# iliasam/STM32F4_SDR_GPS

Hardware: AMD Instinct MI355X
Metric: acquisition hypotheses/sec (PRN x Doppler x phase) (higher is better)
Workload: dtype u1 (MX-FP4 operands, exact f32 accumulation)

## Files before the change

stm32f4_sdr_gps_amd/csrc/k_acq_mx.hip:

```cpp
#if !defined(GPSX_LAB) && defined(MX_VARIANT_B)
#error "variants of k_acq_mx for same-box A/B timing build with -DGPSX_LAB only: tools/build_variant.sh"
#endif
#include <cstdlib>

#include "gpsx_device.hpp"
#include "gpsx_kernels.hpp"

namespace gpsx {

namespace {

typedef int v8i __attribute__((ext_vector_type(8)));
typedef int v4i __attribute__((ext_vector_type(4)));
typedef float v16f __attribute__((ext_vector_type(16)));

constexpr int kMxThreads = 512;
constexpr int kMxTiles = 4;
constexpr int kCopyDwords = 260;
constexpr int kVecDwords = 258;
constexpr int kPlaneWordsMx = 66;
constexpr u32 kScaleOne = 0x7F7F7F7Fu;
constexpr u32 kScaleA = 0x72727272u;
constexpr float kAccScale = 1.0f / 8192.0f;
constexpr float kUnscaleSq = 67108864.0f;
constexpr u32 kScaleEight = 0x82828282u;
constexpr int kPasses = 17;

struct MxShared {
  uint16_t x[1024];
  u32 d[2][514];
  u32 plane[2][16][kPlaneWordsMx];
  u32 base[2][kCopyDwords];
  u32 e8[2][2][8][kCopyDwords];
  u32 corr[2][2][2][128];
  v4i chips_a[16][2][32];
  u32 chip_t[1032];
  u32 ones[2];
  u32 t_lut[768];
  alignas(16) u32 part[8][32][2][32];
};

__device__ __forceinline__ v8i widen(v4i x) { return v8i{x.x, x.y, x.z, x.w, 0, 0, 0, 0}; }

__device__ __forceinline__ u32 lds_byte(const u32 *words, int byte_index)
{
  return (words[byte_index >> 2] >> ((byte_index & 3) * 8)) & 0xFFu;
}

__device__ __forceinline__ u32 spread8(u32 x)
{
  u32 t = (x | (x << 12)) & 0x000F000Fu;
  t = (t | (t << 6)) & 0x03030303u;
  t = (t | (t << 3)) & 0x11111111u;
  return t;
}

__device__ __forceinline__ int wrap1023(int i)
{
  i = i >= 2 * kChips ? i - 2 * kChips : i;
  return i >= kChips ? i - kChips : i;
}

__device__ __forceinline__ u32 plane_bits9(const u32 *pl, int pos)
{
  return __builtin_amdgcn_alignbit(pl[(pos >> 5) + 1], pl[pos >> 5], (u32)(pos & 31)) & 0x1FFu;
}

__device__ __forceinline__ void mx_load_block(MxShared &sh, const uint8_t *blk, int if_format, int tid)
{
  for (int i = tid; i < 1024; i += kMxThreads)
    sh.x[i] = i < kWords16 ? load_sign16(blk, i, if_format) : (uint16_t)0;
  if (tid < 2)
    sh.ones[tid] = 0;
}
__device__ void mx_wipe_block(MxShared &sh, u32 step_word, int tid, int lane)
{
  {
    const u32 *x32 = reinterpret_cast<const u32 *>(sh.x);
    u32 ones_i = 0, ones_q = 0;
    for (int w = tid; w < 514; w += kMxThreads) {
      u32 vi = 0, vq = 0;
      if (w < kWords32) {
        const u32 quad = (step_word * (u32)w) >> 30;
        vi = carrier_i(quad) ^ x32[w];
        vq = carrier_q(quad) ^ x32[w];
      }
      sh.d[0][w] = vi;
      sh.d[1][w] = vq;
      ones_i += __popc(vi);
      ones_q += __popc(vq);
    }
    ones_i = wave_sum_to_lane63(ones_i);
    ones_q = wave_sum_to_lane63(ones_q);
    if (lane == 63) {
      atomicAdd(&sh.ones[0], ones_i);
      atomicAdd(&sh.ones[1], ones_q);
    }
  }
  __syncthreads();
  if (tid < 2)
    sh.d[tid][511] = sh.d[tid][0] << 16;
  __syncthreads();
  for (int m = tid; m < 2 * 32 * 16; m += kMxThreads) {
    const int t0 = m & 15, w = (m >> 4) & 31, iq = m >> 9;
    const u32 *src = &sh.d[iq][16 * w];
    u32 bits = 0;
#pragma unroll
    for (int k = 0; k < 16; k++) {
      const u32 sk = src[k];
      bits |= ((sk >> t0) & 1u) << (2 * k);
      bits |= ((sk >> (16 + t0)) & 1u) << (2 * k + 1);
    }
    sh.plane[iq][t0][w] = bits;
  }
  __syncthreads();
  for (int m = tid; m < 2 * 16 * (kPlaneWordsMx - 32); m += kMxThreads) {
    const int w = 32 + m % (kPlaneWordsMx - 32);
    const int r = m / (kPlaneWordsMx - 32);
    const u32 *pl = sh.plane[r >> 4][r & 15];
    const int pos = 32 * w - (w >= 64 ? 2 * kChips : kChips);
    const int lo = pos >> 5;
    u32 v = __builtin_amdgcn_alignbit(lo < 31 ? pl[lo + 1] : 0u, pl[lo], (u32)(pos & 31));
    if (pos + 32 > kChips) {
      const int k = kChips - pos;
      v = (v & ((1u << k) - 1u)) | (pl[0] << k);
    }
    sh.plane[r >> 4][r & 15][w] = v;
  }
}

__device__ __forceinline__ u32 fp4_code(int v)
{
  const u32 m = (u32)(v < 0 ? -v : v);
  return ((0x0765420u >> (4u * (m > 5u ? 5u : m))) & 0xFu) | (v < 0 ? 8u : 0u);
}

__device__ void mx_fill_tables(MxShared &sh, int tid)
{
  for (int w = tid; w < 512; w += kMxThreads) {
    const u32 cur = (u32)w & 0xFFu, nxt = ((u32)w >> 1) & 0xFFu;
    const u32 plus = spread8(nxt & ~cur), minus = spread8(cur & ~nxt);
    sh.t_lut[w] = (plus << 2) | (plus << 3) | (minus << 2);
  }
  for (int x = tid; x < 256; x += kMxThreads)
    sh.t_lut[512 + x] = (spread8((u32)x) << 1) | (spread8(~(u32)x & 0xFFu) * 0xAu);
}

__device__ void mx_vector_phase1(MxShared &sh, int pass, int buf, int tid, int nthreads)
{
  const int t0 = pass - 1;
  for (int m = tid; m < 2 * kVecDwords + 2 * 128; m += nthreads) {
    if (m < 2 * kVecDwords) {
      const int iq = m >= kVecDwords, dw = m - iq * kVecDwords;
      u32 packed = 0;
      if (pass < 2) {
        const u32 *dd = sh.d[iq];
#pragma unroll
        for (int e = 0; e < 8; e++) {
          const int k = wrap1023(8 * dw + e);
          const int pos = 16 * k;
          const u32 sum = pop16(__builtin_amdgcn_alignbit(dd[(pos >> 5) + 1], dd[pos >> 5], (u32)(pos & 31)));
          const u32 code = pass == 0 ? (0xFEC0u >> (4u * (sum & 3u))) & 0xFu : (0xEDCA0u >> (4u * (sum >> 2))) & 0xFu;
          packed |= code << (4 * e);
        }
      } else {
        const u32 w = plane_bits9(sh.plane[iq][pass - 2], 8 * dw);
        packed = sh.t_lut[w];
        if (dw == 127 && t0 >= 9) {
          const u32 cur = w & 0xFFu, nxt = (w >> 1) & 0xFFu;
          const int e5 = (int)((nxt >> 5) & 1u) - (int)((cur >> 5) & 1u), e6 = (int)((nxt >> 6) & 1u) - (int)((cur >> 6) & 1u);
          packed = (packed & ~0x0FF00000u) | (fp4_code(-2 * e5 - 1) << 20) | (fp4_code(-2 * e6 + 1) << 24);
        }
      }
      sh.base[iq][dw] = packed;
    } else {
      const int mm = m - 2 * kVecDwords;
      const int iq = mm >> 7, dw = mm & 127;
      u32 ca = 0, cb = 0;
      if (pass >= 2 && t0 != 8) {
        const u32 *pl = sh.plane[iq][pass - 2];
        const u32 w = dw ? plane_bits9(pl, 8 * dw - 1) : (pl[0] << 1) & 0x1FFu;
        const u32 exist = dw == 127 ? 0x0FFFFFFFu : 0xFFFFFFFFu;
        if (t0 < 8) {
          ca = sh.t_lut[512 + (w >> 1)] & exist;
        } else {
          const u32 diff = sh.t_lut[w];
          ca = (diff ^ ((diff & 0x44444444u) << 1)) & exist;
          cb = sh.t_lut[512 + (w & 0xFFu)] & exist;
          if (dw == 0) {
            ca = (ca & ~0xFu) | ((w & 2u) ? 0x2u : 0xAu);
            cb &= ~0xFu;
          }
        }
      }
      sh.corr[buf][iq][0][dw] = ca;
      sh.corr[buf][iq][1][dw] = cb;
    }
  }
}

__device__ void mx_vector_phase2(MxShared &sh, int buf, int tid, int nthreads)
{
  for (int m = tid; m < 2 * 256; m += nthreads) {
    const int iq = m >> 8, j = m & 255;
    const u32 lo = sh.base[iq][j], hi = sh.base[iq][j + 1];
#pragma unroll
    for (int c = 0; c < 8; c++)
      sh.e8[buf][iq][c][j] = c ? __builtin_amdgcn_alignbit(hi, lo, 4u * (u32)c) : lo;
  }
}

typedef __attribute__((address_space(3))) const u32 lds_cu32;

__device__ __forceinline__ lds_cu32 *lds_opaque(const u32 *p)
{
  u32 a = (u32)(size_t)(lds_cu32 *)p;
  asm volatile("" : "+v"(a));
  return (lds_cu32 *)(size_t)a;
}
__device__ __forceinline__ v4i lds_frag(lds_cu32 *w, int dw)
{
  return v4i{(int)w[dw], (int)w[dw + 1], (int)w[dw + 2], (int)w[dw + 3]};
}

__device__ __forceinline__ u32 mx_patch_wrap(u32 packed, u32 w9, bool patch)
{
  const u32 i5 = 1u + ((w9 >> 6) & 1u) - ((w9 >> 5) & 1u), i6 = 1u + ((w9 >> 7) & 1u) - ((w9 >> 6) & 1u);
  const u32 c5 = (0xDA2u >> (4u * i5)) & 0xFu;
  const u32 c6 = (0xA25u >> (4u * i6)) & 0xFu;
  const u32 patched = (packed & ~0x0FF00000u) | (c5 << 20) | (c6 << 24);
  return patch ? patched : packed;
}

__device__ __forceinline__ void mx_vector_build(MxShared &sh, int p_vec, int tid)
{
  const int t0 = p_vec - 1, buf = p_vec & 1;
  const bool late = t0 >= 9;
  const int iq = tid >> 8, j = tid & 255, which = (tid >> 7) & 1, dwc = tid & 127;
  const u32 *pl = sh.plane[iq][p_vec - 2];
  const u32 x = __builtin_amdgcn_alignbit(pl[(j >> 2) + 1], pl[j >> 2], 8u * (u32)(j & 3));
  const int pos = dwc ? 8 * dwc - 1 : 0;
  const u32 y = __builtin_amdgcn_alignbit(pl[(pos >> 5) + 1], pl[pos >> 5], (u32)(pos & 31));
  const u32 cw = (dwc ? y : y << 1) & 0x1FFu;
  u32 lo = sh.t_lut[x & 0x1FFu], hi = sh.t_lut[(x >> 8) & 0x1FFu];
  u32 v = sh.t_lut[which ? 512u + (cw & 0xFFu) : (late ? cw : 512u + (cw >> 1))];
  if (late) {
    lo = mx_patch_wrap(lo, x & 0x1FFu, j == 127);
    hi = mx_patch_wrap(hi, (x >> 8) & 0x1FFu, j == 126);
    if (which == 0)
      v ^= (v & 0x44444444u) << 1;
    if (dwc == 0)
      v = (v & ~0xFu) | (which ? 0u : ((cw & 2u) ? 0x2u : 0xAu));
  }
  v &= dwc == 127 ? 0x0FFFFFFFu : 0xFFFFFFFFu;
  if ((which && !late) || t0 == 8)
    v = 0;
  sh.corr[buf][iq][which][dwc] = v;
  u32 *dst = &sh.e8[buf][iq][0][j];
#pragma unroll
  for (int c = 0; c < 8; c++)
    dst[c * kCopyDwords] = c ? __builtin_amdgcn_alignbit(hi, lo, 4u * (u32)c) : lo;
}

__device__ __forceinline__ void mx_vector_build_direct(MxShared &sh, int which, int t0s, u32 *e8_dst, int tid)
{
  const int iq = tid >> 8, j = tid & 255;
  const u32 *dd = sh.d[iq];
  u32 w2[2] = {0, 0};
#pragma unroll
  for (int e = 0; e < 16; e++) {
    const int k = wrap1023(8 * j + e);
    const int pos = 16 * k + t0s;
    const u32 sum = pop16(__builtin_amdgcn_alignbit(dd[(pos >> 5) + 1], dd[pos >> 5], (u32)(pos & 31)));
    const u32 code = which == 0 ? (0xFEC0u >> (4u * (sum & 3u))) & 0xFu : (0xEDCA0u >> (4u * (sum >> 2))) & 0xFu;
    w2[e >> 3] |= code << (4 * (e & 7));
  }
  u32 *dst = e8_dst + (iq * 8) * kCopyDwords + j;
#pragma unroll
  for (int c = 0; c < 8; c++)
    dst[c * kCopyDwords] = c ? __builtin_amdgcn_alignbit(w2[1], w2[0], 4u * (u32)c) : w2[0];
}

template <int S, int NT, u32 SCALE_A = kScaleA>
__device__ __forceinline__ void mx_pass_step(lds_cu32 *wi, lds_cu32 *wq, const v4i *ca, v4i (&a)[16], v4i &fi, v4i &fq,
                                             v16f (&acc)[2][NT], u32 scale_b)
{
  constexpr int kSteps = 16 + NT - 1;
  constexpr bool more = S + 1 < kSteps;
  v4i fi_next = fi, fq_next = fq;
  if constexpr (more) {
    fi_next = lds_frag(wi, 8 * (S + 1));
    fq_next = lds_frag(wq, 8 * (S + 1));
    if constexpr (S + 1 < 16)
      a[S + 1] = ca[(S + 1) * 64];
  }
  constexpr int j_lo = S - 15 > 0 ? S - 15 : 0, j_hi = S < NT - 1 ? S : NT - 1;
#pragma unroll
  for (int j = j_lo; j <= j_hi; j++) {
    acc[0][j] = __builtin_amdgcn_mfma_scale_f32_32x32x64_f8f6f4(widen(a[S - j]), widen(fi), acc[0][j], 4, 4, 0, SCALE_A, 0, scale_b);
    acc[1][j] = __builtin_amdgcn_mfma_scale_f32_32x32x64_f8f6f4(widen(a[S - j]), widen(fq), acc[1][j], 4, 4, 0, SCALE_A, 0, scale_b);
  }
  if constexpr (more) {
    __builtin_amdgcn_sched_group_barrier(0x100, S + 1 < 16 ? 5 : 4, 0);
    __builtin_amdgcn_sched_group_barrier(0x008, 2 * (j_hi - j_lo + 1), 0);
  }
  __builtin_amdgcn_sched_barrier(0);
  fi = fi_next;
  fq = fq_next;
  if constexpr (more)
    mx_pass_step<S + 1, NT, SCALE_A>(wi, wq, ca, a, fi, fq, acc, scale_b);
}

template <int S, int NT>
__device__ __forceinline__ void mx_pass_step_inplace(lds_cu32 *wi, lds_cu32 *wq, const v4i *ca, v4i (&a)[16], v4i &fi, v4i &fq,
                                                     v16f (&acc)[2][NT], u32 scale_b)
{
  constexpr int kSteps = 16 + NT - 1;
  constexpr bool more = S + 1 < kSteps;
  if constexpr (more && S + 1 < 16)
    a[S + 1] = ca[(S + 1) * 64];
  constexpr int j_lo = S - 15 > 0 ? S - 15 : 0, j_hi = S < NT - 1 ? S : NT - 1;
#pragma unroll
  for (int j = j_lo; j <= j_hi; j++)
    acc[0][j] = __builtin_amdgcn_mfma_scale_f32_32x32x64_f8f6f4(widen(a[S - j]), widen(fi), acc[0][j], 4, 4, 0, kScaleA, 0, scale_b);
  if constexpr (more)
    fi = lds_frag(wi, 8 * (S + 1));
#pragma unroll
  for (int j = j_lo; j <= j_hi; j++)
    acc[1][j] = __builtin_amdgcn_mfma_scale_f32_32x32x64_f8f6f4(widen(a[S - j]), widen(fq), acc[1][j], 4, 4, 0, kScaleA, 0, scale_b);
  if constexpr (more)
    fq = lds_frag(wq, 8 * (S + 1));
  if constexpr (more) {
    if constexpr (S + 1 < 16)
      __builtin_amdgcn_sched_group_barrier(0x100, 1, 0);
    __builtin_amdgcn_sched_group_barrier(0x008, j_hi - j_lo + 1, 0);
    __builtin_amdgcn_sched_group_barrier(0x100, 2, 0);
    __builtin_amdgcn_sched_group_barrier(0x008, j_hi - j_lo + 1, 0);
    __builtin_amdgcn_sched_group_barrier(0x100, 2, 0);
  }
  __builtin_amdgcn_sched_barrier(0);
  if constexpr (more)
    mx_pass_step_inplace<S + 1, NT>(wi, wq, ca, a, fi, fq, acc, scale_b);
}

template <int S, int NT>
__device__ __forceinline__ void mx_pass2_step(lds_cu32 *const (&w)[4], const v4i *ca, v4i (&a)[16], v4i (&f)[4], v16f (&acc)[2][NT])
{
  constexpr int kSteps = 16 + NT - 1;
  constexpr bool more = S + 1 < kSteps;
  if constexpr (more && S + 1 < 16)
    a[S + 1] = ca[(S + 1) * 64];
  constexpr int j_lo = S - 15 > 0 ? S - 15 : 0, j_hi = S < NT - 1 ? S : NT - 1;
#pragma unroll
  for (int v = 0; v < 4; v++) {
#pragma unroll
    for (int j = j_lo; j <= j_hi; j++)
      acc[v & 1][j] = __builtin_amdgcn_mfma_scale_f32_32x32x64_f8f6f4(widen(a[S - j]), widen(f[v]), acc[v & 1][j], 4, 4, 0, kScaleA, 0,
                                                                      v < 2 ? kScaleOne : kScaleEight);
    if constexpr (more)
      f[v] = lds_frag(w[v], 8 * (S + 1));
  }
  if constexpr (more) {
    if constexpr (S + 1 < 16)
      __builtin_amdgcn_sched_group_barrier(0x100, 1, 0);
#pragma unroll
    for (int v = 0; v < 4; v++) {
      __builtin_amdgcn_sched_group_barrier(0x008, j_hi - j_lo + 1, 0);
      __builtin_amdgcn_sched_group_barrier(0x100, 2, 0);
    }
  }
  __builtin_amdgcn_sched_barrier(0);
  if constexpr (more)
    mx_pass2_step<S + 1, NT>(w, ca, a, f, acc);
}
template <int NT>
__device__ __forceinline__ void mx_pass2(const MxShared &sh, int lane, int q0_tile, v16f (&acc)[2][NT], const u32 *e8_low,
                                         const u32 *e8_high)
{
  const int n = lane & 31, h = lane >> 5;
  const int off = (n & 7) * kCopyDwords + 4 * (q0_tile + h) + (n >> 3);
  lds_cu32 *const w[4] = {lds_opaque(e8_low + off), lds_opaque(e8_low + 8 * kCopyDwords + off), lds_opaque(e8_high + off),
                          lds_opaque(e8_high + 8 * kCopyDwords + off)};
  const v4i *ca = &sh.chips_a[0][h][n];
  v4i a[16];
  v4i f[4] = {lds_frag(w[0], 0), lds_frag(w[1], 0), lds_frag(w[2], 0), lds_frag(w[3], 0)};
  a[0] = ca[0];
  mx_pass2_step<0, NT>(w, ca, a, f, acc);
}

template <bool AHEAD, int NT, u32 SCALE_A = kScaleA>
__device__ __forceinline__ void mx_pass(const MxShared &sh, int buf, int lane, int q0_tile, v16f (&acc)[2][NT],
                                        u32 scale_b, v4i a_corr, bool with_corr, const u32 *e8_buf = nullptr)
{
  const int n = lane & 31, h = lane >> 5;
  const u32 *e8 = e8_buf ? e8_buf : &sh.e8[buf][0][0][0];
  lds_cu32 *wi = lds_opaque(e8 + (n & 7) * kCopyDwords + 4 * (q0_tile + h) + (n >> 3));
  lds_cu32 *wq = lds_opaque(e8 + (8 + (n & 7)) * kCopyDwords + 4 * (q0_tile + h) + (n >> 3));
  const v4i *ca = &sh.chips_a[0][h][n];
  v4i a[16];
  if constexpr (AHEAD) {
    v4i fi = lds_frag(wi, 0), fq = lds_frag(wq, 0);
    a[0] = ca[0];
    mx_pass_step<0, NT, SCALE_A>(wi, wq, ca, a, fi, fq, acc, scale_b);
  } else {
    static_assert(SCALE_A == kScaleA, "the in-place walk is the sign-only grid's");
    v4i fi = lds_frag(wi, 0), fq = lds_frag(wq, 0);
    a[0] = ca[0];
    mx_pass_step_inplace<0, NT>(wi, wq, ca, a, fi, fq, acc, scale_b);
  }
  if (with_corr) {
    lds_cu32 *cw = lds_opaque(&sh.corr[buf][0][h][4 * q0_tile + (n >> 3)]);
#pragma unroll
    for (int j = 0; j < NT; j++) {
      const v4i gi = v4i{(int)(cw[8 * j] >> (4 * (n & 7))), 0, 0, 0};
      const v4i gq = v4i{(int)(cw[8 * j + 2 * 128] >> (4 * (n & 7))), 0, 0, 0};
      acc[0][j] = __builtin_amdgcn_mfma_scale_f32_32x32x64_f8f6f4(widen(a_corr), widen(gi), acc[0][j], 4, 4, 0, kScaleA, 0,
                                                                   kScaleOne);
      acc[1][j] = __builtin_amdgcn_mfma_scale_f32_32x32x64_f8f6f4(widen(a_corr), widen(gq), acc[1][j], 4, 4, 0, kScaleA, 0,
                                                                   kScaleOne);
    }
  }
}

__device__ __forceinline__ u32 root_trunc(float e);
__device__ __forceinline__ float mx_clip_square(float c)
{
  return __builtin_amdgcn_fmed3f(c * __builtin_fabsf(c), 0.0f, 1.0f);
}
__device__ __forceinline__ float clip_square_sum(float ci, float cq)
{
  return mx_clip_square(ci) + mx_clip_square(cq);
}
__device__ __forceinline__ u32 mag8_f32(float ci, float cq)
{
  return root_trunc(clip_square_sum(ci, cq) * kUnscaleSq);
// ... 440 lines not shown
  const int n = lane & 31, h = lane >> 5;
  const int b = t0 & 7, half = t0 >> 3;
  u32 *slot = &sh.part[slots < 0 ? b : slots][4 * h][0][n];
  u32 best[16], total[16];
  u32 kqh[NT];
#pragma unroll
  for (int j = 0; j < NT; j++)
    kqh[j] = kq[j] - (u32)half;
#pragma unroll
  for (int r = 0; r < 16; r++) {
    best[r] = 0;
    total[r] = 0u - (u32)NT * kRootBias;
  }
  mx_round_toward_zero();
#pragma unroll
  for (int jp = 0; jp < NT; jp += 2) {
#pragma unroll
    for (int r0 = 0; r0 < 16; r0 += 4) {
      float ev[8];
      u32 e_max = 0;
#pragma unroll
      for (int i = 0; i < 8; i++) {
        ev[i] = clip_square_sum(acc[0][jp + (i >> 2)][r0 + (i & 3)], acc[1][jp + (i >> 2)][r0 + (i & 3)]);
        e_max = max(e_max, __float_as_uint(ev[i]));
      }
      const bool small = __builtin_amdgcn_ballot_w64(e_max >= 0x3C800000u ) == 0;
      u32 bits[8];
      if (__builtin_expect(small, 1)) {
#pragma unroll
        for (int i = 0; i < 8; i++)
          bits[i] = root_bits_small(ev[i]);
      } else {
        float ci[8], cq[8];
#pragma unroll
        for (int i = 0; i < 8; i++) {
          ci[i] = acc[0][jp + (i >> 2)][r0 + (i & 3)];
          cq[i] = acc[1][jp + (i >> 2)][r0 + (i & 3)];
        }
        mx_roots_exact<8>(ci, cq, bits);
#pragma unroll
        for (int i = 0; i < 8; i++)
          bits[i] += kRootBias;
      }
#pragma unroll
      for (int rr = 0; rr < 4; rr++) {
        const int r = r0 + rr;
        const u32 k0 = (bits[rr] << 11) | kqh[jp], k1 = (bits[4 + rr] << 11) | kqh[jp + 1];
        best[r] = max(max(best[r], k0), k1);
        total[r] = total[r] + bits[rr] + bits[4 + rr];
      }
#pragma unroll
      for (int rr = 0; rr < 4; rr++)
        asm volatile("" : "+v"(best[r0 + rr]), "+v"(total[r0 + rr]));
      __builtin_amdgcn_sched_barrier(0);
    }
  }
  mx_round_to_nearest();
#pragma unroll
  for (int r = 0; r < 16; r++) {
    const int p_off = ((r & 3) + 8 * (r >> 2)) * 64;
    atomicMax(slot + p_off, best[r]);
    atomicAdd(slot + p_off + 32, total[r]);
  }
}

__device__ __forceinline__ void mx_epilogue_store(int lane, int q0_tile, int t0, const v16f (&acc)[2][kMxTiles], u32 group_mask,
                                                  uint16_t *__restrict__ plane0, size_t prn_stride, int slot0, int n_prn)
{
  const int n = lane & 31, h = lane >> 5;
#pragma unroll
  for (int j = 0; j < kMxTiles; j++) {
    const int q = 32 * (q0_tile + 2 * j) + n;
    uint16_t *v = plane0 + (size_t)t0 * 1024 + (size_t)(q & 3) * 256 + (size_t)(q >> 2);
#pragma unroll
    for (int g = 0; g < 4; g++) {
#pragma unroll
      for (int rr = 0; rr < 4; rr++) {
        const int r = 4 * g + rr;
        const int p = (r & 3) + 8 * (r >> 2) + 4 * h;
        const u32 val = mag8_f32(acc[0][j][r], acc[1][j][r]);
        if (((group_mask >> g) & 1u) && slot0 + p < n_prn)
          v[(size_t)p * prn_stride] = (uint16_t)val;
      }
      __builtin_amdgcn_sched_barrier(0);
    }
  }
}



__device__ __forceinline__ unsigned long long mx_max8_u64(unsigned long long v)
{
  u32 lo = (u32)v, hi = (u32)(v >> 32);
#define MX_MAX8(ctrl)                                                                           \
  {                                                                                             \
    const u32 lo2 = (u32)__builtin_amdgcn_mov_dpp((int)lo, ctrl, 0xF, 0xF, true);               \
    const u32 hi2 = (u32)__builtin_amdgcn_mov_dpp((int)hi, ctrl, 0xF, 0xF, true);               \
    const bool g = hi2 > hi || (hi2 == hi && lo2 > lo);                                         \
    lo = g ? lo2 : lo;                                                                          \
    hi = g ? hi2 : hi;                                                                          \
  }
  MX_MAX8(0xB1)
  MX_MAX8(0x4E)
  MX_MAX8(0x141)
#undef MX_MAX8
  return ((unsigned long long)hi << 32) | lo;
}

constexpr int kMxSingle = 0, kMxWalk = 1, kMxStore = 2, kMxWalk16 = 3, kMxByte = 4, kMxSplit = 5;

}

__global__ void k_build_mx_tables(const u32 *__restrict__ chipbits, int n_slots, u32 *__restrict__ mx_a, u32 *__restrict__ mx_t)
{
  const int n_sets = (n_slots + 31) / 32;
  const int idx = blockIdx.x * blockDim.x + threadIdx.x;
  const int per_set = 16 * 2 * 32 * 4 + 1032;
  if (idx >= n_sets * per_set)
    return;
  const int set = idx / per_set, r = idx - set * per_set;
  if (r < 16 * 2 * 32 * 4) {
    const int dw = r & 3, p = (r >> 2) & 31, h = (r >> 7) & 1, kappa = r >> 8;
    const int slot = 32 * set + p;
    const u32 word = slot < n_slots ? chipbits[(size_t)slot * 32 + 2 * kappa + h] : 0u;
    mx_a[(size_t)set * (16 * 2 * 32 * 4) + r] = spread8((word >> (8 * dw)) & 0xFFu) << 1;
  } else {
    const int c = r - 16 * 2 * 32 * 4 - 1;
    u32 w = 0;
    if (c >= 0 && c < kChips)
      for (int p = 0; p < 32; p++) {
        const int slot = 32 * set + p;
        if (slot < n_slots)
          w |= ((chipbits[(size_t)slot * 32 + (c >> 5)] >> (c & 31)) & 1u) << p;
      }
    mx_t[(size_t)set * 1032 + (c + 1)] = w;
  }
}

void launch_build_mx_tables(hipStream_t s, const uint32_t *d_chipbits, int n_slots, uint32_t *d_mx_a, uint32_t *d_mx_t)
{
  const int n_sets = (n_slots + 31) / 32;
  const int n = n_sets * (16 * 2 * 32 * 4 + 1032);
  hipLaunchKernelGGL(k_build_mx_tables, dim3((n + 255) / 256), dim3(256), 0, s, d_chipbits, n_slots, d_mx_a, d_mx_t);
}

template <int MODE>
__device__ __forceinline__ void mx_unit(MxShared &sh, const AcqParams &prm, int wg, int &tables_set, int cluster_lo,
                                        const uint8_t *__restrict__ if_blocks, const u32 *__restrict__ mx_a,
                                        const u32 *__restrict__ mx_t, gpsx_peak_t *__restrict__ peaks, u32 *__restrict__ energy,
                                        u32 *__restrict__ flags)
{
  constexpr bool MULTI = MODE == kMxWalk || MODE == kMxWalk16, STORE = MODE == kMxStore, S16 = MODE == kMxWalk16;
  constexpr bool SPLIT = MODE == kMxSplit;
  typedef SumRecT<S16> SumRec;
  if constexpr (MODE == kMxWalk) {
    if (flags && flags[wg] == 0)
      return;
  }
  const int tid = threadIdx.x;
  const int lane = tid & 63, wave = __builtin_amdgcn_readfirstlane(tid >> 6);
  const int role = wave >> 2;
  const int q0_tile = 8 * (wave >> 1) + (wave & 1);

  const int n_sets = (prm.n_groups + 3) / 4;
  const int ms_store = STORE ? wg % prm.n_ms : 0;
  const int n_seg = SPLIT ? prm.split_segs : 1;
  const int seg = SPLIT ? wg % n_seg : 0;
  const int cluster = cluster_lo + (STORE ? wg / prm.n_ms : SPLIT ? wg / n_seg : wg);
  const int set = cluster % n_sets;
  const int sd = cluster / n_sets;
  const int dopp = sd % prm.n_dopp;
  const int search = sd / prm.n_dopp;
  u32 group_mask = 0;
#pragma unroll
  for (int g = 0; g < 4; g++) {
    const int group = 4 * set + g;
    const int unit = sd * prm.n_groups + group;
    if (group < prm.n_groups && unit >= prm.unit_lo && unit < prm.unit_hi)
      group_mask |= 1u << g;
  }
  group_mask = (u32)__builtin_amdgcn_readfirstlane((int)group_mask);
  if (group_mask == 0)
    return;
  const float freq_hz = (float)(prm.if_hz + prm.dopp_min_hz + dopp * prm.dopp_step_hz);
  const u32 step_word = nco_step_per_word(freq_hz);

  if (tables_set != set) {
    const u32 *src_a = mx_a + (size_t)set * (16 * 2 * 32 * 4);
    u32 *dst_a = reinterpret_cast<u32 *>(&sh.chips_a[0][0][0]);
    for (int i = tid; i < 16 * 2 * 32 * 4; i += kMxThreads)
      dst_a[i] = src_a[i];
    const u32 *src_t = mx_t + (size_t)set * 1032;
    for (int i = tid; i < 1032; i += kMxThreads)
      sh.chip_t[i] = src_t[i];
    mx_fill_tables(sh, tid);
    tables_set = set;
  }
  for (int i = tid; i < 8 * 32 * 2 * 32 / 4; i += kMxThreads)
    reinterpret_cast<uint4 *>(&sh.part[0][0][0][0])[i] = make_uint4(0, 0, 0, 0);
  const size_t block_bytes = prm.if_format == GPSX_IF_2BIT_SM ? GPSX_BYTES_PER_MS_2BIT : kBytes;
  const uint8_t *block0 = if_blocks + (size_t)(search * prm.search_stride_blocks + (STORE ? wg % prm.n_ms : 0)) * block_bytes;
  mx_load_block(sh, block0, prm.if_format, tid);

  __syncthreads();
  const v4i a_corr = v4i{(int)(((sh.chip_t[(lane >> 5 ? 1021 : 1022) + 1] >> (lane & 31)) & 1u) << 1), 0, 0, 0};
  u32 kq[kMxTiles];
#pragma unroll
  for (int j = 0; j < kMxTiles; j++) {
    kq[j] = (u32)(2047 - 2 * (32 * (q0_tile + 2 * j) + (lane & 31)));
    if constexpr (!MULTI && !STORE)
      asm volatile("" : "+v"(kq[j]));
  }
  u32 *e_wave = MULTI ? energy + ((size_t)wg * 8 + wave) * (16 * kMxTiles * 4 * 64 * (S16 ? 2 : 3)) : nullptr;
  const u32 *zero_recs = MULTI ? flags - kMxZeroRecBytes / sizeof(u32) : nullptr;
  u32 witness = 0;
  const int n_ms = MULTI ? prm.n_ms : 1;
  const int t0s = SPLIT ? seg * (16 / n_seg) : 0;
  const int n_pass = SPLIT ? 16 / n_seg + 1 : kPasses;
  const int pbase = t0s;
#pragma unroll 1
  for (int ms = 0; ms < n_ms; ms++) {
    const bool ms_first = ms == 0, ms_last = ms == n_ms - 1;
    int tid_p = tid, lane_p = lane;
    if constexpr (MULTI)
      asm volatile("" : "+v"(tid_p), "+v"(lane_p));
    if (ms > 0) {
      __syncthreads();
      mx_load_block(sh, block0 + (size_t)ms * block_bytes, prm.if_format, tid_p);
      __syncthreads();
    }
    mx_wipe_block(sh, step_word, tid_p, lane_p);
    if (SPLIT && seg) {
      mx_vector_build_direct(sh, 0, t0s, &sh.e8[0][0][0][0], tid);
      mx_vector_build_direct(sh, 1, t0s, &sh.e8[1][0][0][0], tid);
      for (int i = tid; i < 2 * 2 * 2 * 128; i += kMxThreads)
        (&sh.corr[0][0][0][0])[i] = 0;
    } else {
      __syncthreads();
      mx_vector_phase1(sh, 0, 0, tid_p, kMxThreads);
      __syncthreads();
      mx_vector_phase2(sh, 0, tid_p, kMxThreads);
      __syncthreads();
      mx_vector_phase1(sh, 1, 1, tid_p, kMxThreads);
      __syncthreads();
      mx_vector_phase2(sh, 1, tid_p, kMxThreads);
    }

    v16f acc[2][kMxTiles];
    mx_init_acc(sh.ones, lane_p, q0_tile, acc, prm.win_start, prm.win_stop);
    SumRec pre[MULTI ? 16 : 1];

#pragma unroll 1
    for (int hs = 0; hs <= 2 * n_pass; hs++) {
      if ((hs & 1) == 0)
        __syncthreads();
      constexpr bool kBuildBehindEpilogue = MULTI;
      if (!kBuildBehindEpilogue && (hs & 1) == 0) {
        const int p_vec = (hs >> 1) + 1;
        if (p_vec >= 2 && p_vec < n_pass) {
          int tid_v = tid;
          if constexpr (MULTI)
            asm volatile("" : "+v"(tid_v));
          mx_vector_build(sh, pbase + p_vec, tid_v);
        }
      }
      int lane_s = lane;
      if constexpr (MULTI)
        asm volatile("" : "+v"(lane_s));
      const int x = hs - role;
      const bool active = x >= 0 && x < 2 * n_pass;
      const int p = x >> 1;
      if (active && (x & 1) == 0) {
        if constexpr (MULTI) {
          if (p >= 1)
            mx_prefetch_sums<0, 8, S16>(e_wave, zero_recs, lane_s, p - 1, ms_first, pre);
        }
        mx_pass<!MULTI>(sh, p & 1, lane, q0_tile, acc, p == 1 ? kScaleEight : kScaleOne, a_corr, p >= 2 && (SPLIT || p != 9));
        if constexpr (SPLIT) {
          if (p == 1 && seg) {
            int lane_d = lane;
            asm volatile("" : "+v"(lane_d));
            mx_direct_terms(sh, lane_d, q0_tile, acc, t0s, prm.win_start, prm.win_stop);
          }
        } else {
          if (p == 9)
            mx_half_switch(sh, lane_s, q0_tile, acc, prm.win_start, prm.win_stop);
        }
      }
      if (STORE) {
        if (active && (x & 1) && p >= 1) {
          uint16_t *plane0 = reinterpret_cast<uint16_t *>(energy) +
                             ((size_t)((search * prm.n_ms + ms_store) * prm.n_prn + 32 * set) * prm.n_dopp + dopp) * (16 * 1024);
          mx_epilogue_store(lane, q0_tile, p - 1, acc, group_mask, plane0, (size_t)prm.n_dopp * (16 * 1024), 32 * set, prm.n_prn);
        }
      } else if (active && (x & 1) && p >= 1) {
        if (!MULTI)
          mx_epilogue_single(sh, lane, kq, t0s + p - 1, acc);
        else if (!ms_last)
          mx_epilogue<MULTI, false, S16>(sh, lane_s, q0_tile, p - 1, acc, group_mask, e_wave, zero_recs, pre, ms_first, witness);
        else
          mx_epilogue<MULTI, true, S16>(sh, lane_s, q0_tile, p - 1, acc, group_mask, e_wave, zero_recs, pre, ms_first, witness);
      }
      if (kBuildBehindEpilogue && (x & 1) != 0) {
        const int p_vec = (hs >> 1) + 1;
        if (p_vec >= 2 && p_vec < n_pass) {
          int tid_v = tid;
          if constexpr (MULTI)
            asm volatile("" : "+v"(tid_v));
          mx_vector_build(sh, pbase + p_vec, tid_v);
        }
      }
    }
  }
  if (STORE)
    return;
  if constexpr (S16) {
    if (tid == 0)
      sh.ones[0] = 0;
    __syncthreads();
    if (__builtin_amdgcn_ballot_w64(witness >= 0xFFFFu) != 0 && lane == 0)
      atomicOr(&sh.ones[0], 1u);
  }
  __syncthreads();
  if constexpr (S16) {
    if (tid == 0)
      flags[wg] = sh.ones[0];
    if (sh.ones[0])
      return;
  }
  {
    const int which = tid >> 8, p = (tid >> 3) & 31, b = tid & 7;
    const int slot = 32 * set + p;
    const u32 *row = sh.part[b][p][which];
    u32 vals[32];
#pragma unroll
    for (int l = 0; l < 32; l++)
      vals[l] = row[(l + tid) & 31];
    u32 k = 0, t = 0;
#pragma unroll
    for (int l = 0; l < 32; l++) {
      k = vals[l] > k ? vals[l] : k;
      t += vals[l];
    }
    if (((group_mask >> (p >> 3)) & 1u) && slot < prm.n_prn && b < prm.n_bits) {
      const size_t idx = ((size_t)(search * prm.n_prn + slot) * prm.n_dopp + dopp) * prm.n_bits + b;
      uint2 *pk = reinterpret_cast<uint2 *>(&peaks[idx]);
      if constexpr (SPLIT) {
        const size_t n_planes = (size_t)prm.n_planes;
        if (which == 0)
          atomicMax(&energy[idx], k);
        else
          atomicAdd(&energy[n_planes + idx], t);
      } else if (which == 0) {
        const u32 max_val = k >> 11;
        pk[0] = make_uint2(max_val, max_val ? 2047u - (k & 2047u) : 0u);
      } else {
        pk[1] = make_uint2(t, t / (2u * kChips));
      }
    }
    if constexpr (!SPLIT) {
      if (prm.keys && which == 0) {
        unsigned long long key = 0;
        if (b < prm.n_bits) {
          const u32 max_val = k >> 11, phase = max_val ? 2047u - (k & 2047u) : 0u;
          key = ((unsigned long long)max_val << 14) | (unsigned long long)(16383u - (8u * phase + (u32)b));
        }
        key = mx_max8_u64(key);
        if (b == 0 && ((group_mask >> (p >> 3)) & 1u) && slot < prm.n_prn)
          prm.keys[(size_t)(search * prm.n_prn + slot) * prm.n_dopp + dopp] = (int64_t)key;
      }
    }
  }
}

struct MxBlockRegs {
  u32 v[4];
};
__device__ __forceinline__ MxBlockRegs mx_block_request(const uint8_t *blk, int if_format, int tid)
{
  MxBlockRegs r;
  const uint16_t *p = reinterpret_cast<const uint16_t *>(blk);
  const bool second = 2 * tid + 1 < kWords16;
  if (if_format == GPSX_IF_2BIT_SM) {
    r.v[0] = p[4 * tid];
    r.v[1] = p[4 * tid + 1];
    r.v[2] = second ? p[4 * tid + 2] : 0;
    r.v[3] = second ? p[4 * tid + 3] : 0;
  } else {
    r.v[0] = p[2 * tid];
    r.v[1] = second ? p[2 * tid + 1] : 0;
    r.v[2] = r.v[3] = 0;
  }
  return r;
}
__device__ __forceinline__ void mx_block_commit(MxShared &sh, const MxBlockRegs &r, int if_format, int tid)
{
  u32 lo = r.v[0], hi = r.v[1];
  if (if_format == GPSX_IF_2BIT_SM) {
    lo = even_bits16(r.v[0] | (r.v[1] << 16));
    hi = even_bits16(r.v[2] | (r.v[3] << 16));
  }
  reinterpret_cast<u32 *>(sh.x)[tid] = (lo & 0xFFFFu) | (hi << 16);
}

__device__ __forceinline__ u32 sum_code_low(u32 s) { return (0xFEC0u >> ((s << 2) & 0xCu)) & 0xFu; }
__device__ __forceinline__ u32 sum_code_high(u32 s) { return (0xEDCA0u >> (s & 0x1Cu)) & 0xFu; }
// ... 940 lines not shown
```

Measured before the change: 1283 billion.

## Overlap MX single-mode prologue setup with the first MFMA passes across wave roles

For the single-shot MX mode, the wipe stream now writes the wrap word in place, which removes one barrier. The bit-plane transpose, the second vector build, the LUT fill and the partial-sum zeroing are split between the two wave roles and interleaved with the first two MFMA passes, instead of running serially before the pass loop. A wave-level vector builder uses DPP to get its neighbour codes, and the main loop then starts at a later half-step. The aim is to hide prologue LDS work behind matrix compute. The cost is more complex per-role scheduling, which could introduce LDS hazards or imbalance between roles.

```diff
diff --git a/stm32f4_sdr_gps_amd/csrc/k_acq_mx.hip b/stm32f4_sdr_gps_amd/csrc/k_acq_mx.hip
--- a/stm32f4_sdr_gps_amd/csrc/k_acq_mx.hip
+++ b/stm32f4_sdr_gps_amd/csrc/k_acq_mx.hip
@@ -73,7 +73,8 @@
   if (tid < 2)
     sh.ones[tid] = 0;
 }
-__device__ void mx_wipe_block(MxShared &sh, u32 step_word, int tid, int lane)
+template <bool WRAP_IN_PLACE = false>
+__device__ __forceinline__ void mx_wipe_stream(MxShared &sh, u32 step_word, int tid, int lane)
 {
   {
     const u32 *x32 = reinterpret_cast<const u32 *>(sh.x);
@@ -85,10 +86,14 @@
         vi = carrier_i(quad) ^ x32[w];
         vq = carrier_q(quad) ^ x32[w];
       }
+      ones_i += __popc(vi);
+      ones_q += __popc(vq);
+      if (WRAP_IN_PLACE && w == 511) {
+        vi = (carrier_i(0u) ^ x32[0]) << 16;
+        vq = (carrier_q(0u) ^ x32[0]) << 16;
+      }
       sh.d[0][w] = vi;
       sh.d[1][w] = vq;
-      ones_i += __popc(vi);
-      ones_q += __popc(vq);
     }
     ones_i = wave_sum_to_lane63(ones_i);
     ones_q = wave_sum_to_lane63(ones_q);
@@ -97,9 +102,26 @@
       atomicAdd(&sh.ones[1], ones_q);
     }
   }
-  __syncthreads();
-  if (tid < 2)
-    sh.d[tid][511] = sh.d[tid][0] << 16;
+  if constexpr (!WRAP_IN_PLACE) {
+    __syncthreads();
+    if (tid < 2)
+      sh.d[tid][511] = sh.d[tid][0] << 16;
+  }
+}
+__device__ __forceinline__ u32 mx_plane_ext_word(const u32 *pl, int w)
+{
+  const int pos = 32 * w - (w >= 64 ? 2 * kChips : kChips);
+  const int lo = pos >> 5;
+  u32 v = __builtin_amdgcn_alignbit(lo < 31 ? pl[lo + 1] : 0u, pl[lo], (u32)(pos & 31));
+  if (pos + 32 > kChips) {
+    const int k = kChips - pos;
+    v = (v & ((1u << k) - 1u)) | (pl[0] << k);
+  }
+  return v;
+}
+__device__ void mx_wipe_block(MxShared &sh, u32 step_word, int tid, int lane)
+{
+  mx_wipe_stream(sh, step_word, tid, lane);
   __syncthreads();
   for (int m = tid; m < 2 * 32 * 16; m += kMxThreads) {
     const int t0 = m & 15, w = (m >> 4) & 31, iq = m >> 9;
@@ -117,15 +139,35 @@
   for (int m = tid; m < 2 * 16 * (kPlaneWordsMx - 32); m += kMxThreads) {
     const int w = 32 + m % (kPlaneWordsMx - 32);
     const int r = m / (kPlaneWordsMx - 32);
-    const u32 *pl = sh.plane[r >> 4][r & 15];
-    const int pos = 32 * w - (w >= 64 ? 2 * kChips : kChips);
-    const int lo = pos >> 5;
-    u32 v = __builtin_amdgcn_alignbit(lo < 31 ? pl[lo + 1] : 0u, pl[lo], (u32)(pos & 31));
-    if (pos + 32 > kChips) {
-      const int k = kChips - pos;
-      v = (v & ((1u << k) - 1u)) | (pl[0] << k);
-    }
-    sh.plane[r >> 4][r & 15][w] = v;
+    sh.plane[r >> 4][r & 15][w] = mx_plane_ext_word(sh.plane[r >> 4][r & 15], w);
+  }
+}
+
+__device__ __forceinline__ void mx_planes_half(MxShared &sh, int t0_lo, int v, int lane)
+{
+  const int iq = v >> 1, t0_first = t0_lo + 4 * (v & 1);
+  const int t0 = t0_first + (lane & 3), rot = lane >> 2;
+#pragma unroll 1
+  for (int it = 0; it < 2; it++) {
+    const int w = rot + 16 * it;
+    const u32 *src = &sh.d[iq][16 * w];
+    u32 bits = 0;
+#pragma unroll
+    for (int k = 0; k < 16; k++) {
+      const int kk = (k + rot) & 15;
+      const u32 sk = src[kk];
+      bits |= ((sk >> t0) & 1u) << (2 * kk);
+      bits |= ((sk >> (16 + t0)) & 1u) << (2 * kk + 1);
+    }
+    sh.plane[iq][t0][w] = bits;
+  }
+  __builtin_amdgcn_fence(__ATOMIC_ACQ_REL, "wavefront");
+  asm volatile("s_waitcnt lgkmcnt(0)" ::: "memory");
+#pragma unroll 1
+  for (int m = lane; m < 4 * (kPlaneWordsMx - 32); m += 64) {
+    const int r = m / (kPlaneWordsMx - 32), w = 32 + m % (kPlaneWordsMx - 32);
+    u32 *pl = sh.plane[iq][t0_first + r];
+    pl[w] = mx_plane_ext_word(pl, w);
   }
 }
 
@@ -135,14 +177,14 @@
   return ((0x0765420u >> (4u * (m > 5u ? 5u : m))) & 0xFu) | (v < 0 ? 8u : 0u);
 }
 
-__device__ void mx_fill_tables(MxShared &sh, int tid)
-{
-  for (int w = tid; w < 512; w += kMxThreads) {
+__device__ void mx_fill_tables(MxShared &sh, int tid, int nthreads = kMxThreads)
+{
+  for (int w = tid; w < 512; w += nthreads) {
     const u32 cur = (u32)w & 0xFFu, nxt = ((u32)w >> 1) & 0xFFu;
     const u32 plus = spread8(nxt & ~cur), minus = spread8(cur & ~nxt);
     sh.t_lut[w] = (plus << 2) | (plus << 3) | (minus << 2);
   }
-  for (int x = tid; x < 256; x += kMxThreads)
+  for (int x = tid; x < 256; x += nthreads)
     sh.t_lut[512 + x] = (spread8((u32)x) << 1) | (spread8(~(u32)x & 0xFFu) * 0xAu);
 }
 
@@ -281,6 +323,30 @@
     dst[c * kCopyDwords] = c ? __builtin_amdgcn_alignbit(w2[1], w2[0], 4u * (u32)c) : w2[0];
 }
 
+__device__ __forceinline__ void mx_vector_build_direct_wave(MxShared &sh, int which, int t0s, u32 *e8_dst, int tid)
+{
+  const int iq = tid >> 8, j = tid & 255, l8 = tid & 7;
+  const u32 *dd = sh.d[iq];
+  auto code = [&](int entry) {
+    const int pos = 16 * wrap1023(entry) + t0s;
+    const u32 sum = pop16(__builtin_amdgcn_alignbit(dd[(pos >> 5) + 1], dd[pos >> 5], (u32)(pos & 31)));
+    return which == 0 ? (0xFEC0u >> (4u * (sum & 3u))) & 0xFu : (0xEDCA0u >> (4u * (sum >> 2))) & 0xFu;
+  };
+  u32 lo = 0;
+#pragma unroll
+  for (int e = 0; e < 8; e++)
+    lo |= code(8 * j + e) << (4 * e);
+  u32 above = code(8 * ((j | 63) + 1) + l8) << (4 * l8);
+  above |= dpp<0xB1>(above, above);
+  above |= dpp<0x4E>(above, above);
+  above |= dpp<0x141>(above, above);
+  const u32 hi = dpp<0x130>(above, lo);
+  u32 *dst = e8_dst + (iq * 8) * kCopyDwords + j;
+#pragma unroll
+  for (int c = 0; c < 8; c++)
+    dst[c * kCopyDwords] = c ? __builtin_amdgcn_alignbit(hi, lo, 4u * (u32)c) : lo;
+}
+
 template <int S, int NT, u32 SCALE_A = kScaleA>
 __device__ __forceinline__ void mx_pass_step(lds_cu32 *wi, lds_cu32 *wq, const v4i *ca, v4i (&a)[16], v4i &fi, v4i &fq,
                                              v16f (&acc)[2][NT], u32 scale_b)
@@ -1027,6 +1093,7 @@
 {
   constexpr bool MULTI = MODE == kMxWalk || MODE == kMxWalk16, STORE = MODE == kMxStore, S16 = MODE == kMxWalk16;
   constexpr bool SPLIT = MODE == kMxSplit;
+  constexpr bool SINGLE = MODE == kMxSingle;
   typedef SumRecT<S16> SumRec;
   if constexpr (MODE == kMxWalk) {
     if (flags && flags[wg] == 0)
@@ -1068,11 +1135,14 @@
     const u32 *src_t = mx_t + (size_t)set * 1032;
     for (int i = tid; i < 1032; i += kMxThreads)
       sh.chip_t[i] = src_t[i];
-    mx_fill_tables(sh, tid);
+    if constexpr (!SINGLE)
+      mx_fill_tables(sh, tid);
     tables_set = set;
   }
-  for (int i = tid; i < 8 * 32 * 2 * 32 / 4; i += kMxThreads)
-    reinterpret_cast<uint4 *>(&sh.part[0][0][0][0])[i] = make_uint4(0, 0, 0, 0);
+  if constexpr (!SINGLE) {
+    for (int i = tid; i < 8 * 32 * 2 * 32 / 4; i += kMxThreads)
+      reinterpret_cast<uint4 *>(&sh.part[0][0][0][0])[i] = make_uint4(0, 0, 0, 0);
+  }
   const size_t block_bytes = prm.if_format == GPSX_IF_2BIT_SM ? GPSX_BYTES_PER_MS_2BIT : kBytes;
   const uint8_t *block0 = if_blocks + (size_t)(search * prm.search_stride_blocks + (STORE ? wg % prm.n_ms : 0)) * block_bytes;
   mx_load_block(sh, block0, prm.if_format, tid);
@@ -1104,13 +1174,18 @@
       mx_load_block(sh, block0 + (size_t)ms * block_bytes, prm.if_format, tid_p);
       __syncthreads();
     }
-    mx_wipe_block(sh, step_word, tid_p, lane_p);
-    if (SPLIT && seg) {
+    if constexpr (SINGLE) {
+      mx_wipe_stream<true>(sh, step_word, tid_p, lane_p);
+      __syncthreads();
+      mx_vector_build_direct_wave(sh, 0, 0, &sh.e8[0][0][0][0], tid);
+    } else if (SPLIT && seg) {
+      mx_wipe_block(sh, step_word, tid_p, lane_p);
       mx_vector_build_direct(sh, 0, t0s, &sh.e8[0][0][0][0], tid);
       mx_vector_build_direct(sh, 1, t0s, &sh.e8[1][0][0][0], tid);
       for (int i = tid; i < 2 * 2 * 2 * 128; i += kMxThreads)
         (&sh.corr[0][0][0][0])[i] = 0;
     } else {
+      mx_wipe_block(sh, step_word, tid_p, lane_p);
       __syncthreads();
       mx_vector_phase1(sh, 0, 0, tid_p, kMxThreads);
       __syncthreads();
@@ -1122,11 +1197,38 @@
     }
 
     v16f acc[2][kMxTiles];
-    mx_init_acc(sh.ones, lane_p, q0_tile, acc, prm.win_start, prm.win_stop);
+    if (!SINGLE || role == 0)
+      mx_init_acc(sh.ones, lane_p, q0_tile, acc, prm.win_start, prm.win_stop);
     SumRec pre[MULTI ? 16 : 1];
 
+    if constexpr (SINGLE) {
+      auto opaque = [](int v) {
+        asm volatile("" : "+v"(v));
+        return v;
+      };
+      __syncthreads();
+      if (role) {
+        mx_init_acc(sh.ones, opaque(lane), q0_tile, acc, prm.win_start, prm.win_stop);
+        mx_vector_build_direct_wave(sh, 1, 0, &sh.e8[1][0][0][0], opaque(tid) - 256);
+        mx_vector_build_direct_wave(sh, 1, 0, &sh.e8[1][0][0][0], opaque(tid));
+        mx_fill_tables(sh, opaque(tid) & 255, 256);
+      }
+      mx_pass<true>(sh, 0, lane, q0_tile, acc, kScaleOne, a_corr, false);
+      if (!role) {
+        mx_planes_half(sh, 0, wave, opaque(lane));
+        for (int i = opaque(tid); i < 8 * 32 * 2 * 32 / 4; i += 256)
+          reinterpret_cast<uint4 *>(&sh.part[0][0][0][0])[i] = make_uint4(0, 0, 0, 0);
+      }
+      __syncthreads();
+      mx_vector_build(sh, 2, opaque(tid));
+      if (role)
+        mx_planes_half(sh, 8, wave & 3, opaque(lane));
+      mx_pass<true>(sh, 1, lane, q0_tile, acc, kScaleEight, a_corr, false);
+      if (!role)
+        mx_epilogue_single(sh, lane, kq, 0, acc);
+    }
 #pragma unroll 1
-    for (int hs = 0; hs <= 2 * n_pass; hs++) {
+    for (int hs = SINGLE ? 4 : 0; hs <= 2 * n_pass; hs++) {
       if ((hs & 1) == 0)
         __syncthreads();
       constexpr bool kBuildBehindEpilogue = MULTI;
```

Measured after the change: 1298 billion (median of 6 runs). 1.2% higher.
